# sadit/Jchemo.jl

Measured on AMD Instinct MI355X. Metric: latent-variables/sec (plskern n=1e6 p=500 q=10 nlv=25), higher is better.
Workload: dtype f64

## Files before the change

### jchemo.jl_amd/csrc/fit.hip

```cpp
#include <stdlib.h>
#include <time.h>

#include <algorithm>
#include <condition_variable>
#include <mutex>
#include <thread>

#include "jch_internal.h"

__global__ __launch_bounds__(256) void k_fill_const(double *__restrict__ v, int m, double c)
{
    const int j = blockIdx.x * 256 + threadIdx.x;
    if (j < m) v[j] = c;
}

__global__ __launch_bounds__(256) void k_nan_zero_weight_rows(double *__restrict__ T, int64_t n, int nlv, const double *__restrict__ d)
{
    const int64_t i = (int64_t)blockIdx.x * 256 + threadIdx.x;
    if (i < n && d[i] == 0.0)
        for (int a = 0; a < nlv; ++a) T[(size_t)i + (size_t)a * (size_t)n] = __builtin_nan("");
}

__global__ __launch_bounds__(256) void k_widen_bf16(const unsigned short *__restrict__ src, int64_t ld, int64_t n, int64_t cols, double *__restrict__ dst)
{
// ... 281 lines not shown
        hipEvent_t evb = jch_ev(ctx);
        int nlvb = 0;
        JCH_TRY(jch_fit_plskern_bf16(ctx, d, io.X, io.ldx, io.Y, io.ldy, wdev, dn, Tdev, s, ldr, qpad, ldz, fastb, &nlvb));
        hipEvent_t eve = jch_ev(ctx);
        const size_t ev_last = ctx->ev_used - 1;
        JCH_TRY(fetch_small(nlvb));
        JCH_TRY(jch_p2p_check(ctx));
        if (io.nlv_out) *io.nlv_out = nlvb;
        if (ctx->profiling) {
            jch_profile &pr = ctx->prof;
            pr.fit_ms = ev_ms(evb, eve);
            pr.prologue_ms = ctx->ev_mark > 0 ? ev_ms(evb, ctx->ev_pool[ctx->ev_mark - 1]) : 0.0;
            double sw = 0.0; int cnt = 0;
            for (size_t i = ctx->ev_mark; i + 1 < ev_last; i += 2) { sw += ev_ms(ctx->ev_pool[i], ctx->ev_pool[i + 1]); ++cnt; }
            if (ctx->prof_stride > 1 && cnt > 0 && cnt < nlvb) { sw = sw * (double)nlvb / (double)cnt; cnt = nlvb; }
            pr.sweep_ms = sw; pr.sweep_launches = cnt; pr.nlv = nlvb;
            pr.smallstate_ms = pr.fit_ms - pr.prologue_ms - sw;
            pr.sweep_bytes = (double)n * ((p + 7) & ~7) * 2.0 + 16.0 * (double)n;
            jch_coll_collect(ctx, pr);
        }
        return JCH_OK;
    }
    hipEvent_t ev_begin = jch_ev(ctx);
    JCH_TRY(jch_launch_weights(ctx, wdev, n, dn, s.hdr, qual_dev, 8, mshift_buf, ldr + 2));
    int64_t n_total = n;
    if (ctx->nranks > 1 && n < std::min<int64_t>(p, d.nlv)) {
        double hdr_h[2];
        JCH_HIP(ctx, hipMemcpyAsync(hdr_h, s.hdr, sizeof hdr_h, hipMemcpyDeviceToHost, ctx->stream));
        JCH_HIP(ctx, hipStreamSynchronize(ctx->stream));
        n_total = (int64_t)(hdr_h[1] + 0.5);
    }
    const int nlv = (int)std::min<int64_t>(std::min<int64_t>(n_total, p), d.nlv);
    const bool fast = q <= 16 && nlv <= 1024 && p <= JCH_SWEEP_MAXP && jch_lv_fast_lds_bytes(p, q, qpad, ldr, nlv) <= 150 * 1024;
    const bool sib = algo == ALGO_SIMP || algo == ALGO_WOLD;
    const bool sib_fast = sib && jch_sibling_supported(p, q, ldr, nlv);
    const bool all_fast = sib ? (sib_fast && (algo == ALGO_SIMP || fast)) : fast;
    const int max_slices = all_fast ? JCH_ZT_SLICES : 1;
    const bool fuse_inbox = all_fast && ctx->p2p.ready && !ctx->loop &&
                            (size_t)(ldr + 1 + qpad) <= ctx->p2p.cap;
    int nslice = 1;
    const bool ext_scales = io.xscales_in != nullptr;
    const bool raw_mode = (((algo == ALGO_KERN || algo == ALGO_ROSA) && fast) || (algo == ALGO_SIMP && all_fast)) && !ext_scales && !inplace &&
                          q <= 15 && (d.reserved & ~JCH_REUSE_XCOPY) == 0 && p <= JCH_SWEEP_MAXP && allow_raw && !jch_knob_set("JCH_CENTRED_COPY");
    if (raw_mode) {
        s.mshift = mshift_buf;
        double *spread2 = cv.take(p);
        JCH_TRY(jch_launch_pivot(ctx, Xc, ldxc, n, p, s.hdr, s.scl, spread2));
        JCH_TRY(jch_launch_moments(ctx, Yc, ldyc, nullptr, 0, dn, n, q, 0, nullptr, s.scl + p));
        bool from_copy = false;
        if (reuse_x) JCH_TRY(jch_launch_xty_rows(ctx, Xr, ldr, Yc, ldyc, dn, n, p, q, s.scl, Yr, qpad, s.K, s.mom,
                                                 s.mshift, spread2, qual_dev, s.scl, &from_copy));
        if (from_copy) ctx->xcopy_reused++;
        else {
        JCH_TRY(jch_launch_center_xty(ctx, Xc, ldxc, Yc, ldyc, dn, n, p, q, s.scl, s.mom, false, Xr, ldr, Yr, qpad, s.K, false,
                                      s.mom, s.mshift, spread2, qual_dev, s.scl));
        ctx->xcopy = xkey; ctx->xcopy_valid = true;
        }
        if (d.scal) {
            s.rs = cv.take((size_t)ldr + 2);
            JCH_HIP(ctx, hipMemsetAsync(s.rs, 0, sizeof(double) * ((size_t)ldr + 2), ctx->stream));
            JCH_TRY(jch_launch_raw_scales(ctx, Xr, n, p, ldr, dn, s.mshift, Yr, qpad, q, s.zt, s.scl, s.K));
        }
        s.variant = 2;
    } else {
    ctx->xcopy_valid = false;
    JCH_TRY(jch_launch_moments(ctx, Xc, ldxc, Yc, ldyc, dn, n, p, q, nullptr, s.mom));
    if (ext_scales) {
        JCH_TRY(jch_reserve_host(ctx, sizeof(double) * (size_t)(p + q)));
        double *h = (double *)ctx->hstage;
        for (int j = 0; j < p; ++j) h[j] = io.xscales_in[j];
        for (int k = 0; k < q; ++k) h[p + k] = io.yscales_in ? io.yscales_in[k] : 1.0;
        JCH_HIP(ctx, hipMemcpyAsync(s.scl, h, sizeof(double) * (size_t)(p + q), hipMemcpyHostToDevice, ctx->stream));
        JCH_HIP(ctx, hipStreamSynchronize(ctx->stream));
    } else if (d.scal) JCH_TRY(jch_launch_moments(ctx, Xc, ldxc, Yc, ldyc, dn, n, p, q, s.mom, s.scl));
    else hipLaunchKernelGGL(k_fill_const, dim3((p + q + 255) / 256), dim3(256), 0, ctx->stream, s.scl, p + q, 1.0);
    JCH_TRY(jch_launch_center_xty(ctx, Xc, ldxc, Yc, ldyc, dn, n, p, q, s.mom, s.scl, inplace && kern_like, Xr, ldr, Yr, qpad, s.K, d.scal != 0 || ext_scales));
    }
    hipEvent_t ev_prologue = jch_ev(ctx);
// ... 278 lines not shown
```

### jchemo.jl_amd/csrc/jch_internal.h

```cpp
#pragma once
#include <hip/hip_runtime.h>
#include <stdint.h>
#include <stdio.h>
#include <string.h>

#include <functional>
#include <string>
#include <vector>

#include "jchemo_hip.h"

#define JCH_MAXQ 64
#define JCH_ZT_SLICES 8
#define JCH_SWEEP_MAXP 2048

struct xcopy_key {
    const void *X; int64_t n, ldx; int p, host;
    bool operator==(const xcopy_key &o) const { return X == o.X && n == o.n && ldx == o.ldx && p == o.p && host == o.host; }
};
struct jch_buf {
    void *ptr = nullptr;
    size_t bytes = 0;
};

// ... 135 lines not shown
void jch_coll_begin(jch_ctx *ctx);
void jch_coll_end(jch_ctx *ctx);
void jch_coll_reset(jch_ctx *ctx);
void jch_coll_collect(jch_ctx *ctx, jch_profile &pr);

struct jch_part_view {
    const double *part = nullptr;
    int nb = 0, ldpart = 0;
};

int32_t jch_launch_weights(jch_ctx *ctx, const double *w_dev , int64_t n, double *dnorm,
                           double *hdr , double *zero0 = nullptr, int nzero0 = 0,
                           double *zero1 = nullptr, int nzero1 = 0 );
int32_t jch_launch_moments(jch_ctx *ctx, const double *Xc, int64_t ldx, const double *Yc, int64_t ldy,
                           const double *d, int64_t n, int p, int q, const double *means ,
                           double *out , bool do_sqrt = true);
int32_t jch_launch_center_xty(jch_ctx *ctx, double *Xc, int64_t ldx, double *Yc, int64_t ldy, const double *d,
                              int64_t n, int p, int q, const double *mom, const double *scl, bool writeback,
                              double *Xr, int ldr, double *Yr, int qpad, double *K , bool scal,
                              double *means_out = nullptr ,
                              double *mshift_out = nullptr ,
                              const double *spread2 = nullptr ,
                              double *qual = nullptr ,
                              double *ones_out = nullptr );
int32_t jch_launch_pivot(jch_ctx *ctx, const double *Xc, int64_t ldx, int64_t n, int p, const double *hdr ,
                         double *pivot , double *spread2 );
int32_t jch_launch_export_colmajor(jch_ctx *ctx, const double *Xr, int ldr, const double *Yr, int qpad, int64_t n,
                                   int p, int q, double *Xc, int64_t ldx, double *Yc, int64_t ldy,
                                   const double *sqrt_rowscale = nullptr );
int32_t jch_launch_sweep(jch_ctx *ctx, const double *Xr, int64_t n, int p, int ldr, const double *d, const double *rvec,
                         const double *Yr, int qpad, int q_extra ,
                         double *tcol, double *zt , int ldz, int max_slices,
                         int *nslice_out, const double *mu = nullptr ,
                         jch_part_view *pv = nullptr );
int32_t jch_launch_reduce_rows(jch_ctx *ctx, const double *part, int nb, int ldpart, int m, double *out);
int32_t jch_launch_xty_rows(jch_ctx *ctx, const double *Xr, int ldr, const double *Yc, int64_t ldy, const double *d, int64_t n, int p, int q,
                            const double *mom, double *Yr, int qpad, double *K, double *means_out, double *mshift_out,
                            const double *spread2, double *qual, double *ones_out, bool *done);
int32_t jch_launch_raw_scales(jch_ctx *ctx, const double *Xr, int64_t n, int p, int ldr, const double *d, const double *mshift,
                              const double *Yr, int qpad, int q, double *tmp, double *scl, double *K);
int32_t jch_launch_reduce_part8(jch_ctx *ctx, const double *part, int nb, int ldpart, int m, double *zt, int ldz, int *nslice_out);
int32_t jch_launch_sweep_wide(jch_ctx *ctx, const double *Xr, int64_t n, int ldr, const double *d, const double *rvec,
                              const double *Yr, int qpad, bool nipals, double *tcol, double *zt);
int32_t jch_launch_ytdt(jch_ctx *ctx, const double *Yr, int64_t n, int qpad, const double *d, const double *tcol, double *out );
#define JCH_NIPALS_DEFER_DEFAULT 6
static inline int jch_nipals_lazy_pitch(int ldr) { return 128 * (ldr <= 128 ? 1 : ldr <= 256 ? 2 : ldr <= 512 ? 4 : ldr <= 1024 ? 8 : 16); }
int32_t jch_sweep_tickets(jch_ctx *ctx, int **out);
int jch_nipals_lazy_capacity(int ldr, int q);
int32_t jch_launch_sweep_lazy(jch_ctx *ctx, const double *Xr, int64_t n, int ldr, const double *d, const double *wvec,
                              const double *Yr, int qpad, double *tcol, double *zt, int ldz, int max_slices, int *nslice_out,
                              const double *pend_p, int npend, int npend_max, const double *tpend, int64_t tstride);
int32_t jch_launch_kpass_lazy(jch_ctx *ctx, double *Xr, int64_t n, int p, int ldr, double *Yr, int qpad, int q, const double *d,
                              const double *pend_p, int npend, int npend_max, const double *tpend, int64_t tstride,
                              const double *cvec, bool flush, double *Knext);
int32_t jch_launch_deflate(jch_ctx *ctx, double *Xr, int64_t n, int p, int ldr, double *Yr, int qpad, int q,
                           const double *d, const double *tcol, const double *zpc ,
                           double *Knext );
struct jch_small {
    double *K;
    double *w, *r;
    double *P, *R, *W;
// ... 112 lines not shown
```

### jchemo.jl_amd/csrc/prologue.hip

```cpp
#include <stdint.h>
#include <stdlib.h>

#include <algorithm>

#include "jch_internal.h"
#include "rowsum_dev.h"

typedef double v4f64 __attribute__((ext_vector_type(4)));

__global__ __launch_bounds__(256) void k_wsum_part(const double *__restrict__ w, int64_t n, double *__restrict__ part)
{
    __shared__ double sc[4];
    double s = 0.0;
    for (int64_t i = (int64_t)blockIdx.x * 256 + threadIdx.x; i < n; i += (int64_t)gridDim.x * 256) s += w[i];
    s = jch_block_sum<256>(s, sc);
    if (threadIdx.x == 0) part[blockIdx.x] = s;
}

__global__ __launch_bounds__(256) void k_wsum_final(const double *__restrict__ part, int nb, int64_t n, int have_w,
                                                    double *__restrict__ hdr, double *__restrict__ zero0, int nzero0,
                                                    double *__restrict__ zero1, int nzero1)
{
    __shared__ double sc[4];
    for (int i = threadIdx.x; i < nzero0; i += 256) zero0[i] = 0.0;
// ... 10 lines not shown

__global__ __launch_bounds__(256) void k_wnorm(const double *__restrict__ w, int64_t n, const double *__restrict__ hdr,
                                               double *__restrict__ d)
{
    const double sw = hdr[0];
    for (int64_t i = (int64_t)blockIdx.x * 256 + threadIdx.x; i < n; i += (int64_t)gridDim.x * 256)
        d[i] = (w ? w[i] : 1.0) / sw;
}

int32_t jch_launch_weights(jch_ctx *ctx, const double *w, int64_t n, double *dnorm, double *hdr, double *zero0, int nzero0,
                           double *zero1, int nzero1)
{
    const int nb = (int)std::min<int64_t>(1024, (n + 255) / 256 > 0 ? (n + 255) / 256 : 1);
    JCH_TRY(jch_reserve(ctx, ctx->colpart, sizeof(double) * 4096));
    double *part = (double *)ctx->colpart.ptr;
    if (w) hipLaunchKernelGGL(k_wsum_part, dim3(nb), dim3(256), 0, ctx->stream, w, n, part);
    hipLaunchKernelGGL(k_wsum_final, dim3(1), dim3(256), 0, ctx->stream, part, nb, n, w ? 1 : 0, hdr, zero0, nzero0, zero1, nzero1);
    JCH_TRY(jch_allreduce_f64(ctx, hdr, 2));
    hipLaunchKernelGGL(k_wnorm, dim3(nb), dim3(256), 0, ctx->stream, w, n, hdr, dnorm);
    JCH_HIP(ctx, hipGetLastError());
    return JCH_OK;
}

template <bool VAR>
__global__ __launch_bounds__(256) void k_moments(const double *__restrict__ Xc, int64_t ldx, const double *__restrict__ Yc,
                                                  int64_t ldy, const double *__restrict__ d, int64_t n, int p, int q,
                                                  int64_t chunk, const double *__restrict__ means,
                                                  double *__restrict__ colpart, int aligned16)
{
    __shared__ double sc[4];
    const int j = blockIdx.x;
    const double *col = j < p ? Xc + (size_t)j * (size_t)ldx : Yc + (size_t)(j - p) * (size_t)ldy;
    const int64_t i0 = (int64_t)blockIdx.y * chunk;
    const int64_t i1 = i0 + chunk < n ? i0 + chunk : n;
    const double m = VAR ? means[j] : 0.0;
    double s0 = 0.0, s1 = 0.0, s2 = 0.0, s3 = 0.0;
    if (aligned16) {
        typedef double v2 __attribute__((ext_vector_type(2)));
        int64_t i = i0 + 2 * threadIdx.x;
        for (; i + 1536 + 1 < i1; i += 2048) {
            v2 a0 = __builtin_nontemporal_load(reinterpret_cast<const v2 *>(col + i)), a1 = __builtin_nontemporal_load(reinterpret_cast<const v2 *>(col + i + 512)),
               a2 = __builtin_nontemporal_load(reinterpret_cast<const v2 *>(col + i + 1024)), a3 = __builtin_nontemporal_load(reinterpret_cast<const v2 *>(col + i + 1536));
            const v2 d0 = *reinterpret_cast<const v2 *>(d + i), d1 = *reinterpret_cast<const v2 *>(d + i + 512),
                     d2 = *reinterpret_cast<const v2 *>(d + i + 1024), d3 = *reinterpret_cast<const v2 *>(d + i + 1536);
            if (VAR) { a0 -= m; a1 -= m; a2 -= m; a3 -= m; a0 *= a0; a1 *= a1; a2 *= a2; a3 *= a3; }
            s0 += d0.x * a0.x; s0 += d0.y * a0.y; s1 += d1.x * a1.x; s1 += d1.y * a1.y;
            s2 += d2.x * a2.x; s2 += d2.y * a2.y; s3 += d3.x * a3.x; s3 += d3.y * a3.y;
        }
        for (; i < i1; i += 512) {
            double a0 = col[i], a1 = i + 1 < i1 ? col[i + 1] : 0.0;
            if (VAR) { a0 -= m; a0 *= a0; a1 = i + 1 < i1 ? (a1 - m) * (a1 - m) : 0.0; }
            s0 += d[i] * a0;
            if (i + 1 < i1) s0 += d[i + 1] * a1;
        }
    } else {
    int64_t i = i0 + threadIdx.x;
    for (; i + 768 < i1; i += 1024) {
        double a0 = __builtin_nontemporal_load(col + i), a1 = __builtin_nontemporal_load(col + i + 256),
               a2 = __builtin_nontemporal_load(col + i + 512), a3 = __builtin_nontemporal_load(col + i + 768);
        double d0 = d[i], d1 = d[i + 256], d2 = d[i + 512], d3 = d[i + 768];
        if (VAR) { a0 -= m; a1 -= m; a2 -= m; a3 -= m; a0 *= a0; a1 *= a1; a2 *= a2; a3 *= a3; }
        s0 += d0 * a0; s1 += d1 * a1; s2 += d2 * a2; s3 += d3 * a3;
    }
    for (; i < i1; i += 256) {
        double a0 = col[i];
        if (VAR) { a0 -= m; a0 *= a0; }
        s0 += d[i] * a0;
    }
    }
    double s = jch_block_sum<256>((s0 + s1) + (s2 + s3), sc);
    if (threadIdx.x == 0) colpart[(size_t)blockIdx.y * (size_t)(p + q) + j] = s;
}

__global__ __launch_bounds__(256) void k_colreduce(const double *__restrict__ colpart, int S, int m, int sqrt_out,
                                                   double *__restrict__ out)
{
    const int j = blockIdx.x * 256 + threadIdx.x;
    if (j >= m) return;
    double s = 0.0;
    for (int k0 = 0; k0 < S; k0 += 16) {
        double v[16];
#pragma unroll
        for (int u = 0; u < 16; ++u) v[u] = colpart[(size_t)min(k0 + u, S - 1) * m + j];
#pragma unroll
        for (int u = 0; u < 16; ++u) s += k0 + u < S ? v[u] : 0.0;
    }
    out[j] = s;
    (void)sqrt_out;
}

__global__ __launch_bounds__(256) void k_sqrt_inplace(double *__restrict__ v, int m)
{
    const int j = blockIdx.x * 256 + threadIdx.x;
    if (j < m) v[j] = sqrt(v[j]);
}

int32_t jch_launch_moments(jch_ctx *ctx, const double *Xc, int64_t ldx, const double *Yc, int64_t ldy, const double *d,
                           int64_t n, int p, int q, const double *means, double *out, bool do_sqrt)
{
    const int m = p + q;
    int S = (ctx->cus * 8 + m - 1) / m;
    if (S < 1) S = 1;
    if (S > 64) S = 64;
    int64_t chunk = (n + S - 1) / S;
    chunk = (chunk + 255) / 256 * 256;
    if (chunk < 256) chunk = 256;
    S = (int)((n + chunk - 1) / chunk);
    if (S < 1) S = 1;
    JCH_TRY(jch_reserve(ctx, ctx->colpart, sizeof(double) * (size_t)S * m + 4096 * sizeof(double)));
    double *colpart = (double *)ctx->colpart.ptr;
    const int al16 = (ldx % 2 == 0) && ((uintptr_t)Xc % 16 == 0) && (q == 0 || ((ldy % 2 == 0) && ((uintptr_t)Yc % 16 == 0))) &&
                     ((uintptr_t)d % 16 == 0);
    if (means)
        hipLaunchKernelGGL(k_moments<true>, dim3(m, S), dim3(256), 0, ctx->stream, Xc, ldx, Yc, ldy, d, n, p, q, chunk,
                           means, colpart, al16);
    else
        hipLaunchKernelGGL(k_moments<false>, dim3(m, S), dim3(256), 0, ctx->stream, Xc, ldx, Yc, ldy, d, n, p, q, chunk,
                           means, colpart, al16);
    hipLaunchKernelGGL(k_colreduce, dim3((m + 255) / 256), dim3(256), 0, ctx->stream, colpart, S, m, 0, out);
    JCH_TRY(jch_allreduce_f64(ctx, out, (size_t)m));
    if (means && do_sqrt) hipLaunchKernelGGL(k_sqrt_inplace, dim3((m + 255) / 256), dim3(256), 0, ctx->stream, out, m);
    JCH_HIP(ctx, hipGetLastError());
    return JCH_OK;
}

#define XT_LD 65
#define YT_LD 17
template <bool WRITEBACK, bool SCAL>
__global__ __launch_bounds__(256) void k_center_xty(double *__restrict__ Xc, int64_t ldx, const double *__restrict__ Yc,
                                                     int64_t ldy, const double *__restrict__ d, int64_t n, int p, int q,
                                                     const double *__restrict__ mom, const double *__restrict__ scl,
// ... 18 lines not shown
    auto prefetch = [&](int64_t cc) {
        const int64_t i = cc * 64 + lane;
#pragma unroll
        for (int k = 0; k < 16; ++k) {
            const int j = j0 + wv + 4 * k;
            xr[k] = (i < n && j < p) ? __builtin_nontemporal_load(Xc + (size_t)i + (size_t)j * (size_t)ldx) : 0.0;
        }
    };
    int64_t c = blockIdx.x;
    if (c < nchunks) prefetch(c);
    for (; c < nchunks; c += gridDim.x) {
        const int64_t i0 = c * 64;
#pragma unroll
        for (int k = 0; k < 4; ++k) {
            const int e = tid + 256 * k, row = e & 63, col = e >> 6;
            const int yc = yg * 16 + col;
            const int64_t i = i0 + row;
            double v = 0.0, dv = 0.0;
            if (i < n && yc < q) {
                v = Yc[(size_t)i + (size_t)yc * (size_t)ldy] - mom[p + yc];
                if (SCAL) v /= scl[p + yc];
                dv = d[i];
            }
            if (blockIdx.y == 0 && i < n) Yr[(size_t)i * qpad + yc] = v;
            yt[row * YT_LD + col] = (yc == ones_col && i < n) ? d[i] : dv * v;
        }
        {
            const int64_t i = i0 + lane;
#pragma unroll
            for (int k = 0; k < 16; ++k) {
                const int j = j0 + wv + 4 * k;
                double v = 0.0;
                if (i < n && j < p) {
                    v = SCAL ? (xr[k] - cm[k]) / cs[k] : xr[k] - cm[k];
                    if (WRITEBACK && yg == 0) Xc[(size_t)i + (size_t)j * (size_t)ldx] = v;
                }
                xt[lane * XT_LD + wv + 4 * k] = v;
            }
        }
        __syncthreads();
        if (c + gridDim.x < nchunks) prefetch(c + gridDim.x);
        if (yg == 0) {
#pragma unroll 4
            for (int k = 0; k < 16; ++k) {
                const int row = wv + 4 * k, j = j0 + lane;
                const int64_t i = i0 + row;
                if (i < n && j < ldr) __builtin_nontemporal_store(xt[row * XT_LD + lane], Xr + (size_t)i * ldr + j);
// ... 84 lines not shown
        {
            constexpr int NB = BLDS ? TH / 16 : TH / 4;
            double yraw[NB], draw[NB];
            const int yc_ = min(ycol, q - 1);
#pragma unroll
            for (int kq = 0; kq < NB; ++kq) {
                const int kk = BLDS ? wv * (TH / 16) + kq : kq;
                const int64_t row = min(i0 + 4 * kk + (lane >> 4), rend - 1);
                draw[kq] = d[row];
                yraw[kq] = Yc[(size_t)row + (size_t)yc_ * (size_t)ldy];
            }
#pragma unroll
            for (int kq = 0; kq < NB; ++kq) {
                const int kk = BLDS ? wv * (TH / 16) + kq : kq;
                const int64_t row = i0 + 4 * kk + (lane >> 4);
                const bool ok = row < rend;
                double yv = 0.0;
                if (ycol < q) {
                    yv = yraw[kq] - ym;
                    if (SCAL) yv /= ysd;
                }
                const double dv = ok ? draw[kq] : 0.0;
                if (!ok) yv = 0.0;
                if (ok && (BLDS || wv == 0) && blockIdx.y == 0) Yr[(size_t)row * 16 + ycol] = yv;
                const double bv = ycol == ones_col ? dv : dv * yv;
                if (BLDS) yt_s[(4 * kk + (lane >> 4)) * 16 + ycol] = bv;
                else breg[kq] = bv;
            }
        }
#pragma unroll 1
        for (int ct0 = 0; ct0 < ntile; ct0 += NSUB) {
#pragma unroll
            for (int sub = 0; sub < NSUB; ++sub) {
                const int ct = ct0 + sub;
                {
                    const int64_t i = i0 + 2 * rp;
                    const bool ok0 = i < rend, ok1 = i + 1 < rend;
                    const int cb = CPI * wv + csub;
#pragma unroll
                    for (int k = 0; k < NL; ++k) {
                        const int c = cb + 4 * CPI * k;
                        const int j = cg0 + 64 * ct + c;
                        const bool live = ct < ntile && j < p;
                        const double m = cm_s[(64 * ct + c) & 511];
                        v2f64p v = R[k];
                        if (SCAL) { const double sdv = cs_s[(64 * ct + c) & 511]; v.x = (v.x - m) / sdv; v.y = (v.y - m) / sdv; }
                        else { v.x -= m; v.y -= m; }
// ... 50 lines not shown
                                if (dbg_skip & 4) *reinterpret_cast<v2f64p *>(dst + (size_t)(RPI * sidx) * (size_t)ldr) = v;
                                else __builtin_nontemporal_store(v, reinterpret_cast<v2f64p *>(dst + (size_t)(RPI * sidx) * (size_t)ldr));
                            }
                        }
                    }
                    __syncthreads();
                }
            }
        }
    }
    double *kp = Kpart + ((size_t)blockIdx.x * kp_rows) * 16;
#pragma unroll
    for (int ct = 0; ct < 8; ++ct)
        if (ct < ntile) {
#pragma unroll
            for (int reg = 0; reg < 4; ++reg) {
                const int j = cg0 + 64 * ct + 16 * wv + (lane >> 4) + 4 * reg;
                if (j < kp_rows) kp[(size_t)j * 16 + (lane & 15)] = acc[ct][reg];
            }
        }
}

__global__ __launch_bounds__(256) void k_reduce_kpart_wide(const double *__restrict__ Kpart, int nbx, int kp_rows, int p, int qpad,
                                                           double *__restrict__ K)
{
    __shared__ double sc[4][64];
    const int el = threadIdx.x & 63, g = threadIdx.x >> 6;
    const int e = blockIdx.x * 64 + el;
    const size_t stride = (size_t)kp_rows * qpad;
    double s0 = 0.0, s1 = 0.0, s2 = 0.0, s3 = 0.0;
    if (e < p * qpad) {
        int b = g;
        for (; b + 12 < nbx; b += 16) {
            s0 += Kpart[(size_t)b * stride + e]; s1 += Kpart[(size_t)(b + 4) * stride + e];
            s2 += Kpart[(size_t)(b + 8) * stride + e]; s3 += Kpart[(size_t)(b + 12) * stride + e];
        }
        for (; b < nbx; b += 4) s0 += Kpart[(size_t)b * stride + e];
    }
    sc[g][el] = (s0 + s1) + (s2 + s3);
    __syncthreads();
    if (g == 0 && e < p * qpad) K[e] = (sc[0][el] + sc[1][el]) + (sc[2][el] + sc[3][el]);
}

__global__ __launch_bounds__(256) void k_reduce_kpart(const double *__restrict__ Kpart, int nbx, int kp_rows, int p, int qpad,
                                                      double *__restrict__ K)
{
    const int e = blockIdx.x * 256 + threadIdx.x;
    if (e >= p * qpad) return;
    const size_t stride = (size_t)kp_rows * qpad;
    double s = 0.0;
    for (int b = 0; b < nbx; ++b) s += Kpart[(size_t)b * stride + e];
    K[e] = s;
}

__global__ __launch_bounds__(256) void k_extract_means(double *__restrict__ K, int qpad, int p, int col, const double *pivot,
                                                       double *__restrict__ means, double *__restrict__ mshift,
                                                       const double *__restrict__ spread2, double *__restrict__ qual, int q,
                                                       double *ones_out)
{
    const int j = blockIdx.x * 256 + threadIdx.x;
    const double pv = j < p + q ? pivot[j] : 0.0;
    if (ones_out && j >= p && j < p + q) { means[j] = pv; ones_out[j] = 1.0; }
    if (j < p) {
        const double dm = K[(size_t)j * qpad + col];
        means[j] = pv + dm;
        mshift[j] = dm;
        K[(size_t)j * qpad + col] = 0.0;
        if (ones_out) ones_out[j] = 1.0;
        if (qual) {
            const double a = fabs(dm);
            const double ratio = a > 0.0 ? a / sqrt(spread2[j]) : 0.0;
            atomicMax(reinterpret_cast<unsigned long long *>(qual), (unsigned long long)__double_as_longlong(ratio));
        }
    }
}

__global__ __launch_bounds__(256) void k_pivot_rows(const double *__restrict__ Xc, int64_t ldx, int64_t n, int p,
                                                    const double *__restrict__ hdr, double *__restrict__ pivot,
                                                    double *__restrict__ spread2)
{
    const int lane = threadIdx.x & 63, j = blockIdx.x * 4 + (threadIdx.x >> 6);
    if (j >= p) return;
    const int m = (int)(n < 256 ? n : 256);
    const int64_t stride = n / m;
    double v[4], s = 0.0;
#pragma unroll
    for (int k = 0; k < 4; ++k) {
        const int i = lane + 64 * k;
        v[k] = i < m ? Xc[(size_t)i * (size_t)stride + (size_t)j * (size_t)ldx] : 0.0;
        s += v[k];
    }
    const double mean = jch_wave_sum(s) / m;
    double s2 = 0.0;
#pragma unroll
    for (int k = 0; k < 4; ++k) {
        const double e = lane + 64 * k < m ? v[k] - mean : 0.0;
        s2 += e * e;
    }
    s2 = jch_wave_sum(s2) / m;
    const double f = (double)n / hdr[1];
    if (lane == 0) { pivot[j] = mean * f; spread2[j] = s2 * f; }
}

int32_t jch_launch_pivot(jch_ctx *ctx, const double *Xc, int64_t ldx, int64_t n, int p, const double *hdr, double *pivot, double *spread2)
{
    hipLaunchKernelGGL(k_pivot_rows, dim3((p + 3) / 4), dim3(256), 0, ctx->stream, Xc, ldx, n, p, hdr, pivot, spread2);
    JCH_HIP(ctx, hipGetLastError());
    JCH_TRY(jch_allreduce_f64(ctx, pivot, (size_t)p));
    return jch_allreduce_f64(ctx, spread2, (size_t)p);
}

typedef double v2f64r __attribute__((ext_vector_type(2)));
template <int KC, int NQ>
__global__ __launch_bounds__(256) void k_xty_rows(const double *__restrict__ Xr, int64_t n, int ldr, const double *__restrict__ Yc, int64_t ldy,
                                                  const double *__restrict__ d, int q, const double *__restrict__ ymeans, int ones_col,
                                                  double *__restrict__ Yr, double *__restrict__ Kpart, int kp_rows)
{
    extern __shared__ __attribute__((aligned(16))) double xr_red[];
    constexpr int R = 4, NBUF = 3;
    const int lane = threadIdx.x & 63, wv = threadIdx.x >> 6;
    int coff[KC];
#pragma unroll
    for (int k = 0; k < KC; ++k) { const int col = 2 * lane + 128 * k; coff[k] = col < ldr ? col : ldr - 2; }
    v2f64r acc[KC][NQ];
#pragma unroll
    for (int k = 0; k < KC; ++k)
#pragma unroll
        for (int c = 0; c < NQ; ++c) acc[k][c] = v2f64r{0.0, 0.0};
    const int64_t ngroups = (n + R - 1) / R, gstride = (int64_t)gridDim.x * 4;
    const int yk = lane & 15, yr = lane >> 4;
    const double ym = yk < q ? ymeans[yk] : 0.0;
    v2f64r X[NBUF][R][KC];
    double Yv[NBUF], Dv[NBUF];
    auto fetch = [&](int b, int64_t gg) {
        const int64_t r0 = gg * R;
#pragma unroll
        for (int rr = 0; rr < R; ++rr) {
            const int64_t row = r0 + rr < n ? r0 + rr : n - 1;
            const double *rp = Xr + (size_t)row * (size_t)ldr;
#pragma unroll
            for (int k = 0; k < KC; ++k) X[b][rr][k] = __builtin_nontemporal_load(reinterpret_cast<const v2f64r *>(rp + coff[k]));
        }
        const int64_t myrow = r0 + yr < n ? r0 + yr : n - 1;
        Yv[b] = Yc[(size_t)myrow + (size_t)min(yk, q - 1) * (size_t)ldy];
        Dv[b] = d[myrow];
    };
    int64_t g = (int64_t)blockIdx.x * 4 + wv;
#pragma unroll
    for (int b = 0; b < NBUF - 1; ++b)
        if (g + b * gstride < ngroups) fetch(b, g + b * gstride);
    auto process = [&](int b, int64_t gg) {
        const int64_t r0 = gg * R;
        const bool live = r0 + yr < n;
        const double yc = (live && yk < q) ? Yv[b] - ym : 0.0;
        const double dv = live ? Dv[b] : 0.0;
        if (live) Yr[(size_t)(r0 + yr) * 16 + yk] = yc;
        const double bv = yk == ones_col ? dv : dv * yc;
#pragma unroll
        for (int rr = 0; rr < R; ++rr) {
#pragma unroll
            for (int c = 0; c < NQ; ++c) {
                const double bc = jch_readlane(bv, 16 * rr + c);
#pragma unroll
                for (int k = 0; k < KC; ++k) { acc[k][c].x += X[b][rr][k].x * bc; acc[k][c].y += X[b][rr][k].y * bc; }
            }
        }
    };
    while (g < ngroups) {
#pragma unroll
        for (int b = 0; b < NBUF; ++b) {
            if (g < ngroups) {
                const int64_t ahead = g + (NBUF - 1) * gstride;
                if (ahead < ngroups) fetch((b + NBUF - 1) % NBUF, ahead);
                process(b, g);
                g += gstride;
            }
        }
    }
    double *kp = Kpart + (size_t)blockIdx.x * kp_rows * 16;
#pragma unroll 1
    for (int c = 0; c < 16; ++c) {
        if (c < NQ) {
#pragma unroll
            for (int k = 0; k < KC; ++k) {
                v2f64r v = acc[k][0];
#pragma unroll
                for (int cc = 1; cc < NQ; ++cc) v = c == cc ? acc[k][cc] : v;
                *reinterpret_cast<v2f64r *>(xr_red + wv * (KC * 128) + 2 * lane + 128 * k) = v;
            }
        }
        __syncthreads();
        for (int j = threadIdx.x; j < kp_rows; j += 256) {
            double t = 0.0;
            if (c < NQ && j < ldr) t = ((xr_red[j] + xr_red[KC * 128 + j]) + xr_red[2 * KC * 128 + j]) + xr_red[3 * KC * 128 + j];
            kp[(size_t)j * 16 + c] = t;
        }
        __syncthreads();
    }
}

int32_t jch_launch_xty_rows(jch_ctx *ctx, const double *Xr, int ldr, const double *Yc, int64_t ldy, const double *d, int64_t n, int p, int q,
                            const double *mom, double *Yr, int qpad, double *K, double *means_out, double *mshift_out,
                            const double *spread2, double *qual, double *ones_out, bool *done)
{
    *done = false;
    if (qpad != 16 || q + 1 > 12 || ldr > 512 || ldr < 2 || !means_out) return JCH_OK;
    const int ones_col = q;
    const int kc = (ldr + 127) / 128, kp_rows = 512;
    const int64_t ngroups = (n + 3) / 4;
    const int nbx = (int)std::max<int64_t>(1, std::min<int64_t>((ngroups + 3) / 4, ctx->cus));
    JCH_TRY(jch_reserve(ctx, ctx->kpart, sizeof(double) * (size_t)nbx * kp_rows * 16));
    double *Kpart = (double *)ctx->kpart.ptr;
    const int nq = q + 1 <= 4 ? 4 : (q + 1 <= 8 ? 8 : 12);
#define JCH_XR(KC, NQ) hipLaunchKernelGGL((k_xty_rows<KC, NQ>), dim3(nbx), dim3(256), sizeof(double) * 4 * KC * 128, ctx->stream, Xr, n, ldr, Yc, ldy, d, q, \
                                          mom + p, ones_col, Yr, Kpart, kp_rows)
#define JCH_XR_NQ(KC) do { if (nq == 4) JCH_XR(KC, 4); else if (nq == 8) JCH_XR(KC, 8); else JCH_XR(KC, 12); } while (0)
    if (kc == 1) JCH_XR_NQ(1); else if (kc == 2) JCH_XR_NQ(2); else if (kc == 3) JCH_XR_NQ(3); else JCH_XR_NQ(4);
#undef JCH_XR_NQ
#undef JCH_XR
    hipLaunchKernelGGL(k_reduce_kpart_wide, dim3((p * 16 + 63) / 64), dim3(256), 0, ctx->stream, Kpart, nbx, kp_rows, p, 16, K);
    JCH_TRY(jch_allreduce_f64(ctx, K, (size_t)p * qpad));
    hipLaunchKernelGGL(k_extract_means, dim3((p + q + 255) / 256), dim3(256), 0, ctx->stream, K, qpad, p, ones_col, mom, means_out, mshift_out, spread2, qual, q, ones_out);
    JCH_HIP(ctx, hipGetLastError());
    *done = true;
    return JCH_OK;
}

int32_t jch_launch_center_xty(jch_ctx *ctx, double *Xc, int64_t ldx, double *Yc, int64_t ldy, const double *d, int64_t n,
                              int p, int q, const double *mom, const double *scl, bool writeback, double *Xr, int ldr,
                              double *Yr, int qpad, double *K, bool scal, double *means_out, double *mshift_out,
                              const double *spread2, double *qual, double *ones_out)
{
    const int ones_col = means_out ? q : -1;
    if (qpad == 16 && ldx % 2 == 0 && ((uintptr_t)Xc) % 16 == 0) {
        const int groups = (ldr + 511) / 512;
        const int kp_rows = groups * 512;
        const int64_t nunits = (n + 31) / 32;
        int nbx = std::max(1, ctx->cus / groups);
        if (nbx > nunits) nbx = (int)nunits;
        JCH_TRY(jch_reserve(ctx, ctx->kpart, sizeof(double) * (size_t)nbx * kp_rows * 16));
        double *Kpart = (double *)ctx->kpart.ptr;
        dim3 grid(nbx, groups);
        const size_t lds = sizeof(double) * (64 * (64 + 2) + 1024);
#define JCH_K2P(WB, SC) hipLaunchKernelGGL((k_center_xty_panel<64, 64, WB, SC>), grid, dim3(256), lds, ctx->stream, Xc, ldx, Yc, ldy, d, n, p, q, \
                                           mom, scl, Xr, ldr, Yr, Kpart, kp_rows, ones_col, 0)
        if (writeback && scal) JCH_K2P(true, true); else if (writeback) JCH_K2P(true, false);
        else if (scal) JCH_K2P(false, true); else JCH_K2P(false, false);
#undef JCH_K2P
        hipLaunchKernelGGL(k_reduce_kpart_wide, dim3((p * 16 + 63) / 64), dim3(256), 0, ctx->stream, Kpart, nbx, kp_rows, p, 16, K);
        JCH_TRY(jch_allreduce_f64(ctx, K, (size_t)p * qpad));
        if (means_out) hipLaunchKernelGGL(k_extract_means, dim3((p + q + 255) / 256), dim3(256), 0, ctx->stream, K, qpad, p, ones_col, mom, means_out, mshift_out, spread2, qual, q, ones_out);
        JCH_HIP(ctx, hipGetLastError());
        if (writeback)
            JCH_TRY(jch_launch_export_colmajor(ctx, nullptr, ldr, Yr, qpad, n, p, q, Xc, ldx, Yc, ldy));
        return JCH_OK;
    }
    const int tw = 64, th = 64;
    const int ptiles = (ldr + tw - 1) / tw;
    const int kp_rows = ptiles * tw;
    const int ygroups = qpad / 16;
    const int64_t nchunks = (n + th - 1) / th;
    int nbx = (ctx->cus * 3 + ptiles * ygroups - 1) / (ptiles * ygroups);
    if (nbx < 1) nbx = 1;
    if (nbx > nchunks) nbx = (int)(nchunks > 0 ? nchunks : 1);
    const int nslots = nbx;
    JCH_TRY(jch_reserve(ctx, ctx->kpart, sizeof(double) * (size_t)nslots * kp_rows * qpad));
    double *Kpart = (double *)ctx->kpart.ptr;
    dim3 grid(nbx, ptiles, ygroups);
    const bool wb_fused = writeback && ygroups == 1;
#define JCH_K2(WB, SC) hipLaunchKernelGGL((k_center_xty<WB, SC>), grid, dim3(256), 0, ctx->stream, Xc, ldx, Yc, ldy, d, n, p, q, \
                                          mom, scl, Xr, ldr, Yr, qpad, Kpart, kp_rows, ones_col)
    if (wb_fused && scal) JCH_K2(true, true);
    else if (wb_fused) JCH_K2(true, false);
    else if (scal) JCH_K2(false, true);
// ... 62 lines not shown
```

Baseline: 1544.

## Fuse fit prologue kernels and fold mean extraction into K reduction

```diff
diff --git a/jchemo.jl_amd/csrc/fit.hip b/jchemo.jl_amd/csrc/fit.hip
--- a/jchemo.jl_amd/csrc/fit.hip
+++ b/jchemo.jl_amd/csrc/fit.hip
@@ -327,7 +327,10 @@
         return JCH_OK;
     }
     hipEvent_t ev_begin = jch_ev(ctx);
-    JCH_TRY(jch_launch_weights(ctx, wdev, n, dn, s.hdr, qual_dev, 8, mshift_buf, ldr + 2));
+    const bool lean_knob = jch_knob("JCH_FIT_HEAD", 1) != 0;
+    const bool lean = ctx->nranks == 1 && lean_knob;
+    const bool head_fused = lean && !wdev;
+    if (!head_fused) JCH_TRY(jch_launch_weights(ctx, wdev, n, dn, s.hdr, qual_dev, 8, mshift_buf, ldr + 2));
     int64_t n_total = n;
     if (ctx->nranks > 1 && n < std::min<int64_t>(p, d.nlv)) {
         double hdr_h[2];
@@ -347,18 +350,24 @@
     const bool ext_scales = io.xscales_in != nullptr;
     const bool raw_mode = (((algo == ALGO_KERN || algo == ALGO_ROSA) && fast) || (algo == ALGO_SIMP && all_fast)) && !ext_scales && !inplace &&
                           q <= 15 && (d.reserved & ~JCH_REUSE_XCOPY) == 0 && p <= JCH_SWEEP_MAXP && allow_raw && !jch_knob_set("JCH_CENTRED_COPY");
+    if (head_fused && !raw_mode) JCH_TRY(jch_launch_weights(ctx, wdev, n, dn, s.hdr, qual_dev, 8, mshift_buf, ldr + 2));
     if (raw_mode) {
         s.mshift = mshift_buf;
         double *spread2 = cv.take(p);
+        if (head_fused) JCH_TRY(jch_launch_fit_head(ctx, Xc, ldxc, Yc, ldyc, n, p, q, dn, s.hdr, qual_dev, 8, mshift_buf, ldr + 2, s.scl, spread2, s.scl + p));
+        else {
         JCH_TRY(jch_launch_pivot(ctx, Xc, ldxc, n, p, s.hdr, s.scl, spread2));
         JCH_TRY(jch_launch_moments(ctx, Yc, ldyc, nullptr, 0, dn, n, q, 0, nullptr, s.scl + p));
+        }
+        const bool need_yr = d.scal != 0 || !lean_knob;
+        double *Yr_w = need_yr ? Yr : nullptr;
         bool from_copy = false;
-        if (reuse_x) JCH_TRY(jch_launch_xty_rows(ctx, Xr, ldr, Yc, ldyc, dn, n, p, q, s.scl, Yr, qpad, s.K, s.mom,
-                                                 s.mshift, spread2, qual_dev, s.scl, &from_copy));
+        if (reuse_x) JCH_TRY(jch_launch_xty_rows(ctx, Xr, ldr, Yc, ldyc, dn, n, p, q, s.scl, Yr_w, qpad, s.K, s.mom,
+                                                 s.mshift, spread2, qual_dev, s.scl, &from_copy, lean));
         if (from_copy) ctx->xcopy_reused++;
         else {
-        JCH_TRY(jch_launch_center_xty(ctx, Xc, ldxc, Yc, ldyc, dn, n, p, q, s.scl, s.mom, false, Xr, ldr, Yr, qpad, s.K, false,
-                                      s.mom, s.mshift, spread2, qual_dev, s.scl));
+        JCH_TRY(jch_launch_center_xty(ctx, Xc, ldxc, Yc, ldyc, dn, n, p, q, s.scl, s.mom, false, Xr, ldr, Yr_w, qpad, s.K, false,
+                                      s.mom, s.mshift, spread2, qual_dev, s.scl, lean));
         ctx->xcopy = xkey; ctx->xcopy_valid = true;
         }
         if (d.scal) {
diff --git a/jchemo.jl_amd/csrc/jch_internal.h b/jchemo.jl_amd/csrc/jch_internal.h
--- a/jchemo.jl_amd/csrc/jch_internal.h
+++ b/jchemo.jl_amd/csrc/jch_internal.h
@@ -181,7 +181,10 @@
                               double *mshift_out = nullptr ,
                               const double *spread2 = nullptr ,
                               double *qual = nullptr ,
-                              double *ones_out = nullptr );
+                              double *ones_out = nullptr ,
+                              bool fold_means = false );
+int32_t jch_launch_fit_head(jch_ctx *ctx, const double *Xc, int64_t ldx, const double *Yc, int64_t ldy, int64_t n, int p, int q, double *dnorm,
+                            double *hdr, double *zero0, int nzero0, double *zero1, int nzero1, double *pivot, double *spread2, double *ymeans);
 int32_t jch_launch_pivot(jch_ctx *ctx, const double *Xc, int64_t ldx, int64_t n, int p, const double *hdr ,
                          double *pivot , double *spread2 );
 int32_t jch_launch_export_colmajor(jch_ctx *ctx, const double *Xr, int ldr, const double *Yr, int qpad, int64_t n,
@@ -195,7 +198,7 @@
 int32_t jch_launch_reduce_rows(jch_ctx *ctx, const double *part, int nb, int ldpart, int m, double *out);
 int32_t jch_launch_xty_rows(jch_ctx *ctx, const double *Xr, int ldr, const double *Yc, int64_t ldy, const double *d, int64_t n, int p, int q,
                             const double *mom, double *Yr, int qpad, double *K, double *means_out, double *mshift_out,
-                            const double *spread2, double *qual, double *ones_out, bool *done);
+                            const double *spread2, double *qual, double *ones_out, bool *done, bool fold_means = false);
 int32_t jch_launch_raw_scales(jch_ctx *ctx, const double *Xr, int64_t n, int p, int ldr, const double *d, const double *mshift,
                               const double *Yr, int qpad, int q, double *tmp, double *scl, double *K);
 int32_t jch_launch_reduce_part8(jch_ctx *ctx, const double *part, int nb, int ldpart, int m, double *zt, int ldz, int *nslice_out);
diff --git a/jchemo.jl_amd/csrc/prologue.hip b/jchemo.jl_amd/csrc/prologue.hip
--- a/jchemo.jl_amd/csrc/prologue.hip
+++ b/jchemo.jl_amd/csrc/prologue.hip
@@ -56,18 +56,10 @@
     return JCH_OK;
 }
 
-template <bool VAR>
-__global__ __launch_bounds__(256) void k_moments(const double *__restrict__ Xc, int64_t ldx, const double *__restrict__ Yc,
-                                                  int64_t ldy, const double *__restrict__ d, int64_t n, int p, int q,
-                                                  int64_t chunk, const double *__restrict__ means,
-                                                  double *__restrict__ colpart, int aligned16)
-{
-    __shared__ double sc[4];
-    const int j = blockIdx.x;
-    const double *col = j < p ? Xc + (size_t)j * (size_t)ldx : Yc + (size_t)(j - p) * (size_t)ldy;
-    const int64_t i0 = (int64_t)blockIdx.y * chunk;
-    const int64_t i1 = i0 + chunk < n ? i0 + chunk : n;
-    const double m = VAR ? means[j] : 0.0;
+template <bool VAR, bool CONSTD>
+__device__ __forceinline__ double jch_moments_block(const double *__restrict__ col, const double *__restrict__ d, double dc, int64_t i0, int64_t i1,
+                                                    double m, int aligned16, double *sc)
+{
     double s0 = 0.0, s1 = 0.0, s2 = 0.0, s3 = 0.0;
     if (aligned16) {
         typedef double v2 __attribute__((ext_vector_type(2)));
@@ -75,8 +67,9 @@
         for (; i + 1536 + 1 < i1; i += 2048) {
             v2 a0 = __builtin_nontemporal_load(reinterpret_cast<const v2 *>(col + i)), a1 = __builtin_nontemporal_load(reinterpret_cast<const v2 *>(col + i + 512)),
                a2 = __builtin_nontemporal_load(reinterpret_cast<const v2 *>(col + i + 1024)), a3 = __builtin_nontemporal_load(reinterpret_cast<const v2 *>(col + i + 1536));
-            const v2 d0 = *reinterpret_cast<const v2 *>(d + i), d1 = *reinterpret_cast<const v2 *>(d + i + 512),
-                     d2 = *reinterpret_cast<const v2 *>(d + i + 1024), d3 = *reinterpret_cast<const v2 *>(d + i + 1536);
+            const v2 dcv = {dc, dc};
+            const v2 d0 = CONSTD ? dcv : *reinterpret_cast<const v2 *>(d + i), d1 = CONSTD ? dcv : *reinterpret_cast<const v2 *>(d + i + 512),
+                     d2 = CONSTD ? dcv : *reinterpret_cast<const v2 *>(d + i + 1024), d3 = CONSTD ? dcv : *reinterpret_cast<const v2 *>(d + i + 1536);
             if (VAR) { a0 -= m; a1 -= m; a2 -= m; a3 -= m; a0 *= a0; a1 *= a1; a2 *= a2; a3 *= a3; }
             s0 += d0.x * a0.x; s0 += d0.y * a0.y; s1 += d1.x * a1.x; s1 += d1.y * a1.y;
             s2 += d2.x * a2.x; s2 += d2.y * a2.y; s3 += d3.x * a3.x; s3 += d3.y * a3.y;
@@ -84,25 +77,40 @@
         for (; i < i1; i += 512) {
             double a0 = col[i], a1 = i + 1 < i1 ? col[i + 1] : 0.0;
             if (VAR) { a0 -= m; a0 *= a0; a1 = i + 1 < i1 ? (a1 - m) * (a1 - m) : 0.0; }
-            s0 += d[i] * a0;
-            if (i + 1 < i1) s0 += d[i + 1] * a1;
+            s0 += (CONSTD ? dc : d[i]) * a0;
+            if (i + 1 < i1) s0 += (CONSTD ? dc : d[i + 1]) * a1;
         }
     } else {
     int64_t i = i0 + threadIdx.x;
     for (; i + 768 < i1; i += 1024) {
         double a0 = __builtin_nontemporal_load(col + i), a1 = __builtin_nontemporal_load(col + i + 256),
                a2 = __builtin_nontemporal_load(col + i + 512), a3 = __builtin_nontemporal_load(col + i + 768);
-        double d0 = d[i], d1 = d[i + 256], d2 = d[i + 512], d3 = d[i + 768];
+        const double d0 = CONSTD ? dc : d[i], d1 = CONSTD ? dc : d[i + 256], d2 = CONSTD ? dc : d[i + 512], d3 = CONSTD ? dc : d[i + 768];
         if (VAR) { a0 -= m; a1 -= m; a2 -= m; a3 -= m; a0 *= a0; a1 *= a1; a2 *= a2; a3 *= a3; }
         s0 += d0 * a0; s1 += d1 * a1; s2 += d2 * a2; s3 += d3 * a3;
     }
     for (; i < i1; i += 256) {
         double a0 = col[i];
         if (VAR) { a0 -= m; a0 *= a0; }
-        s0 += d[i] * a0;
-    }
-    }
-    double s = jch_block_sum<256>((s0 + s1) + (s2 + s3), sc);
+        s0 += (CONSTD ? dc : d[i]) * a0;
+    }
+    }
+    return jch_block_sum<256>((s0 + s1) + (s2 + s3), sc);
+}
+
+template <bool VAR>
+__global__ __launch_bounds__(256) void k_moments(const double *__restrict__ Xc, int64_t ldx, const double *__restrict__ Yc,
+                                                  int64_t ldy, const double *__restrict__ d, int64_t n, int p, int q,
+                                                  int64_t chunk, const double *__restrict__ means,
+                                                  double *__restrict__ colpart, int aligned16)
+{
+    __shared__ double sc[4];
+    const int j = blockIdx.x;
+    const double *col = j < p ? Xc + (size_t)j * (size_t)ldx : Yc + (size_t)(j - p) * (size_t)ldy;
+    const int64_t i0 = (int64_t)blockIdx.y * chunk;
+    const int64_t i1 = i0 + chunk < n ? i0 + chunk : n;
+    const double m = VAR ? means[j] : 0.0;
+    const double s = jch_moments_block<VAR, false>(col, d, 0.0, i0, i1, m, aligned16, sc);
     if (threadIdx.x == 0) colpart[(size_t)blockIdx.y * (size_t)(p + q) + j] = s;
 }
 
@@ -129,10 +137,8 @@
     if (j < m) v[j] = sqrt(v[j]);
 }
 
-int32_t jch_launch_moments(jch_ctx *ctx, const double *Xc, int64_t ldx, const double *Yc, int64_t ldy, const double *d,
-                           int64_t n, int p, int q, const double *means, double *out, bool do_sqrt)
-{
-    const int m = p + q;
+static void moments_geometry(const jch_ctx *ctx, int64_t n, int m, int *S_out, int64_t *chunk_out)
+{
     int S = (ctx->cus * 8 + m - 1) / m;
     if (S < 1) S = 1;
     if (S > 64) S = 64;
@@ -141,6 +147,15 @@
     if (chunk < 256) chunk = 256;
     S = (int)((n + chunk - 1) / chunk);
     if (S < 1) S = 1;
+    *S_out = S; *chunk_out = chunk;
+}
+
+int32_t jch_launch_moments(jch_ctx *ctx, const double *Xc, int64_t ldx, const double *Yc, int64_t ldy, const double *d,
+                           int64_t n, int p, int q, const double *means, double *out, bool do_sqrt)
+{
+    const int m = p + q;
+    int S; int64_t chunk;
+    moments_geometry(ctx, n, m, &S, &chunk);
     JCH_TRY(jch_reserve(ctx, ctx->colpart, sizeof(double) * (size_t)S * m + 4096 * sizeof(double)));
     double *colpart = (double *)ctx->colpart.ptr;
     const int al16 = (ldx % 2 == 0) && ((uintptr_t)Xc % 16 == 0) && (q == 0 || ((ldy % 2 == 0) && ((uintptr_t)Yc % 16 == 0))) &&
@@ -205,7 +220,7 @@
                 if (SCAL) v /= scl[p + yc];
                 dv = d[i];
             }
-            if (blockIdx.y == 0 && i < n) Yr[(size_t)i * qpad + yc] = v;
+            if (Yr && blockIdx.y == 0 && i < n) Yr[(size_t)i * qpad + yc] = v;
             yt[row * YT_LD + col] = (yc == ones_col && i < n) ? d[i] : dv * v;
         }
         {
@@ -336,7 +351,7 @@
                 }
                 const double dv = ok ? draw[kq] : 0.0;
                 if (!ok) yv = 0.0;
-                if (ok && (BLDS || wv == 0) && blockIdx.y == 0) Yr[(size_t)row * 16 + ycol] = yv;
+                if (Yr && ok && (BLDS || wv == 0) && blockIdx.y == 0) Yr[(size_t)row * 16 + ycol] = yv;
                 const double bv = ycol == ones_col ? dv : dv * yv;
                 if (BLDS) yt_s[(4 * kk + (lane >> 4)) * 16 + ycol] = bv;
                 else breg[kq] = bv;
@@ -433,7 +448,9 @@
 }
 
 __global__ __launch_bounds__(256) void k_reduce_kpart_wide(const double *__restrict__ Kpart, int nbx, int kp_rows, int p, int qpad,
-                                                           double *__restrict__ K)
+                                                           double *__restrict__ K, int col, const double *pivot, double *__restrict__ means,
+                                                           double *__restrict__ mshift, const double *__restrict__ spread2,
+                                                           double *__restrict__ qual, int q, double *ones_out)
 {
     __shared__ double sc[4][64];
     const int el = threadIdx.x & 63, g = threadIdx.x >> 6;
@@ -450,7 +467,27 @@
     }
     sc[g][el] = (s0 + s1) + (s2 + s3);
     __syncthreads();
-    if (g == 0 && e < p * qpad) K[e] = (sc[0][el] + sc[1][el]) + (sc[2][el] + sc[3][el]);
+    if (g == 0 && e < p * qpad) {
+        const double v = (sc[0][el] + sc[1][el]) + (sc[2][el] + sc[3][el]);
+        const int j = e / qpad;
+        if (means && e - j * qpad == col) {
+            const double pv = pivot[j];
+            means[j] = pv + v;
+            mshift[j] = v;
+            K[e] = 0.0;
+            if (ones_out) ones_out[j] = 1.0;
+            if (qual) {
+                const double a = fabs(v);
+                const double ratio = a > 0.0 ? a / sqrt(spread2[j]) : 0.0;
+                atomicMax(reinterpret_cast<unsigned long long *>(qual), (unsigned long long)__double_as_longlong(ratio));
+            }
+        } else K[e] = v;
+    }
+    if (means && ones_out && blockIdx.x == 0 && (int)threadIdx.x < q) {
+        const int j = p + threadIdx.x;
+        const double pv = pivot[j];
+        means[j] = pv; ones_out[j] = 1.0;
+    }
 }
 
 __global__ __launch_bounds__(256) void k_reduce_kpart(const double *__restrict__ Kpart, int nbx, int kp_rows, int p, int qpad,
@@ -486,11 +523,10 @@
     }
 }
 
-__global__ __launch_bounds__(256) void k_pivot_rows(const double *__restrict__ Xc, int64_t ldx, int64_t n, int p,
-                                                    const double *__restrict__ hdr, double *__restrict__ pivot,
-                                                    double *__restrict__ spread2)
-{
-    const int lane = threadIdx.x & 63, j = blockIdx.x * 4 + (threadIdx.x >> 6);
+__device__ __forceinline__ void jch_pivot_block(const double *__restrict__ Xc, int64_t ldx, int64_t n, int p, double n_total, int blk,
+                                                double *__restrict__ pivot, double *__restrict__ spread2)
+{
+    const int lane = threadIdx.x & 63, j = blk * 4 + (threadIdx.x >> 6);
     if (j >= p) return;
     const int m = (int)(n < 256 ? n : 256);
     const int64_t stride = n / m;
@@ -509,8 +545,15 @@
         s2 += e * e;
     }
     s2 = jch_wave_sum(s2) / m;
-    const double f = (double)n / hdr[1];
+    const double f = (double)n / n_total;
     if (lane == 0) { pivot[j] = mean * f; spread2[j] = s2 * f; }
+}
+
+__global__ __launch_bounds__(256) void k_pivot_rows(const double *__restrict__ Xc, int64_t ldx, int64_t n, int p,
+                                                    const double *__restrict__ hdr, double *__restrict__ pivot,
+                                                    double *__restrict__ spread2)
+{
+    jch_pivot_block(Xc, ldx, n, p, hdr[1], blockIdx.x, pivot, spread2);
 }
 
 int32_t jch_launch_pivot(jch_ctx *ctx, const double *Xc, int64_t ldx, int64_t n, int p, const double *hdr, double *pivot, double *spread2)
@@ -519,6 +562,71 @@
     JCH_HIP(ctx, hipGetLastError());
     JCH_TRY(jch_allreduce_f64(ctx, pivot, (size_t)p));
     return jch_allreduce_f64(ctx, spread2, (size_t)p);
+}
+
+__global__ __launch_bounds__(256) void k_fit_head(const double *__restrict__ Yc, int64_t ldy, int64_t n, int q, int64_t chunk, int aligned16,
+                                                  double *__restrict__ colpart, int nb_mom, double nd, double *__restrict__ d, int nb_w,
+                                                  const double *__restrict__ Xc, int64_t ldx, int p, double *__restrict__ pivot,
+                                                  double *__restrict__ spread2)
+{
+    __shared__ double sc[4];
+    int b = blockIdx.x;
+    if (b < nb_mom) {
+        const int j = b % q, sl = b / q;
+        const int64_t i0 = (int64_t)sl * chunk;
+        const int64_t i1 = i0 + chunk < n ? i0 + chunk : n;
+        const double s = jch_moments_block<false, true>(Yc + (size_t)j * (size_t)ldy, nullptr, 1.0 / nd, i0, i1, 0.0, aligned16, sc);
+        if (threadIdx.x == 0) colpart[(size_t)sl * (size_t)q + j] = s;
+        return;
+    }
+    b -= nb_mom;
+    if (b < nb_w) {
+        for (int64_t i = (int64_t)b * 256 + threadIdx.x; i < n; i += (int64_t)nb_w * 256) d[i] = 1.0 / nd;
+        return;
+    }
+    jch_pivot_block(Xc, ldx, n, p, nd, b - nb_w, pivot, spread2);
+}
+
+__global__ __launch_bounds__(256) void k_fit_head_finish(const double *__restrict__ colpart, int S, int q, double *__restrict__ ymeans, double nd,
+                                                         double *__restrict__ hdr, double *__restrict__ zero0, int nzero0,
+                                                         double *__restrict__ zero1, int nzero1)
+{
+    if (blockIdx.x == 0) {
+        for (int i = threadIdx.x; i < nzero0; i += 256) zero0[i] = 0.0;
+        for (int i = threadIdx.x; i < nzero1; i += 256) zero1[i] = 0.0;
+        if (threadIdx.x == 0) { hdr[0] = nd; hdr[1] = nd; }
+    }
+    const int j = blockIdx.x * 256 + threadIdx.x;
+    if (j >= q) return;
+    double s = 0.0;
+    for (int k0 = 0; k0 < S; k0 += 16) {
+        double v[16];
+#pragma unroll
+        for (int u = 0; u < 16; ++u) v[u] = colpart[(size_t)min(k0 + u, S - 1) * q + j];
+#pragma unroll
+        for (int u = 0; u < 16; ++u) s += k0 + u < S ? v[u] : 0.0;
+    }
+    ymeans[j] = s;
+}
+
+int32_t jch_launch_fit_head(jch_ctx *ctx, const double *Xc, int64_t ldx, const double *Yc, int64_t ldy, int64_t n, int p, int q, double *dnorm,
+                            double *hdr, double *zero0, int nzero0, double *zero1, int nzero1, double *pivot, double *spread2, double *ymeans)
+{
+    if (ctx->nranks != 1) return jch_fail(ctx, JCH_EINVAL, "internal: the fused fit head is for one rank");
+    int S; int64_t chunk;
+    moments_geometry(ctx, n, q, &S, &chunk);
+    JCH_TRY(jch_reserve(ctx, ctx->colpart, sizeof(double) * (size_t)S * q + 4096 * sizeof(double)));
+    const int al16 = (ldy % 2 == 0) && ((uintptr_t)Yc % 16 == 0) && ((uintptr_t)dnorm % 16 == 0);
+    const int nb_mom = q * S;
+    const int nb_w = (int)std::min<int64_t>(1024, (n + 255) / 256 > 0 ? (n + 255) / 256 : 1);
+    const int nb_piv = (p + 3) / 4;
+    double *colpart = (double *)ctx->colpart.ptr;
+    hipLaunchKernelGGL(k_fit_head, dim3(nb_mom + nb_w + nb_piv), dim3(256), 0, ctx->stream, Yc, ldy, n, q, chunk, al16, colpart, nb_mom, (double)n,
+                       dnorm, nb_w, Xc, ldx, p, pivot, spread2);
+    hipLaunchKernelGGL(k_fit_head_finish, dim3((q + 255) / 256), dim3(256), 0, ctx->stream, colpart, S, q, ymeans, (double)n, hdr, zero0, nzero0,
+                       zero1, nzero1);
+    JCH_HIP(ctx, hipGetLastError());
+    return JCH_OK;
 }
 
 typedef double v2f64r __attribute__((ext_vector_type(2)));
@@ -565,7 +673,7 @@
         const bool live = r0 + yr < n;
         const double yc = (live && yk < q) ? Yv[b] - ym : 0.0;
         const double dv = live ? Dv[b] : 0.0;
-        if (live) Yr[(size_t)(r0 + yr) * 16 + yk] = yc;
+        if (Yr && live) Yr[(size_t)(r0 + yr) * 16 + yk] = yc;
         const double bv = yk == ones_col ? dv : dv * yc;
 #pragma unroll
         for (int rr = 0; rr < R; ++rr) {
@@ -612,7 +720,7 @@
 
 int32_t jch_launch_xty_rows(jch_ctx *ctx, const double *Xr, int ldr, const double *Yc, int64_t ldy, const double *d, int64_t n, int p, int q,
                             const double *mom, double *Yr, int qpad, double *K, double *means_out, double *mshift_out,
-                            const double *spread2, double *qual, double *ones_out, bool *done)
+                            const double *spread2, double *qual, double *ones_out, bool *done, bool fold_means)
 {
     *done = false;
     if (qpad != 16 || q + 1 > 12 || ldr > 512 || ldr < 2 || !means_out) return JCH_OK;
@@ -629,9 +737,11 @@
     if (kc == 1) JCH_XR_NQ(1); else if (kc == 2) JCH_XR_NQ(2); else if (kc == 3) JCH_XR_NQ(3); else JCH_XR_NQ(4);
 #undef JCH_XR_NQ
 #undef JCH_XR
-    hipLaunchKernelGGL(k_reduce_kpart_wide, dim3((p * 16 + 63) / 64), dim3(256), 0, ctx->stream, Kpart, nbx, kp_rows, p, 16, K);
+    const bool fold = fold_means && ctx->nranks == 1 && q < 256;
+    hipLaunchKernelGGL(k_reduce_kpart_wide, dim3((p * 16 + 63) / 64), dim3(256), 0, ctx->stream, Kpart, nbx, kp_rows, p, 16, K, ones_col, mom,
+                       fold ? means_out : nullptr, mshift_out, spread2, qual, q, ones_out);
     JCH_TRY(jch_allreduce_f64(ctx, K, (size_t)p * qpad));
-    hipLaunchKernelGGL(k_extract_means, dim3((p + q + 255) / 256), dim3(256), 0, ctx->stream, K, qpad, p, ones_col, mom, means_out, mshift_out, spread2, qual, q, ones_out);
+    if (!fold) hipLaunchKernelGGL(k_extract_means, dim3((p + q + 255) / 256), dim3(256), 0, ctx->stream, K, qpad, p, ones_col, mom, means_out, mshift_out, spread2, qual, q, ones_out);
     JCH_HIP(ctx, hipGetLastError());
     *done = true;
     return JCH_OK;
@@ -640,7 +750,7 @@
 int32_t jch_launch_center_xty(jch_ctx *ctx, double *Xc, int64_t ldx, double *Yc, int64_t ldy, const double *d, int64_t n,
                               int p, int q, const double *mom, const double *scl, bool writeback, double *Xr, int ldr,
                               double *Yr, int qpad, double *K, bool scal, double *means_out, double *mshift_out,
-                              const double *spread2, double *qual, double *ones_out)
+                              const double *spread2, double *qual, double *ones_out, bool fold_means)
 {
     const int ones_col = means_out ? q : -1;
     if (qpad == 16 && ldx % 2 == 0 && ((uintptr_t)Xc) % 16 == 0) {
@@ -658,9 +768,11 @@
         if (writeback && scal) JCH_K2P(true, true); else if (writeback) JCH_K2P(true, false);
         else if (scal) JCH_K2P(false, true); else JCH_K2P(false, false);
 #undef JCH_K2P
-        hipLaunchKernelGGL(k_reduce_kpart_wide, dim3((p * 16 + 63) / 64), dim3(256), 0, ctx->stream, Kpart, nbx, kp_rows, p, 16, K);
+        const bool fold = means_out && fold_means && ctx->nranks == 1 && q < 256;
+        hipLaunchKernelGGL(k_reduce_kpart_wide, dim3((p * 16 + 63) / 64), dim3(256), 0, ctx->stream, Kpart, nbx, kp_rows, p, 16, K, ones_col, mom,
+                           fold ? means_out : nullptr, mshift_out, spread2, qual, q, ones_out);
         JCH_TRY(jch_allreduce_f64(ctx, K, (size_t)p * qpad));
-        if (means_out) hipLaunchKernelGGL(k_extract_means, dim3((p + q + 255) / 256), dim3(256), 0, ctx->stream, K, qpad, p, ones_col, mom, means_out, mshift_out, spread2, qual, q, ones_out);
+        if (means_out && !fold) hipLaunchKernelGGL(k_extract_means, dim3((p + q + 255) / 256), dim3(256), 0, ctx->stream, K, qpad, p, ones_col, mom, means_out, mshift_out, spread2, qual, q, ones_out);
         JCH_HIP(ctx, hipGetLastError());
         if (writeback)
             JCH_TRY(jch_launch_export_colmajor(ctx, nullptr, ldr, Yr, qpad, n, p, q, Xc, ldx, Yc, ldy));
```

New measurement: 1543. About the same (-0.1%).
